# vdorie/stan4bart

Hardware: AMD Instinct MI355X
Metric: gibbs_iters_per_sec (higher is better)
Workload: dtype f64

## Files before the change

### include/stan4bart_amd.h

```cpp
#ifndef STAN4BART_AMD_H
#define STAN4BART_AMD_H

#include <stdint.h>
#include <stddef.h>

#ifndef S4B_PREFIX
#define S4B_PREFIX s4b_
#endif
#define S4B_CAT_(a, b) a##b
#define S4B_CAT(a, b) S4B_CAT_(a, b)
#define S4B_FN(name) S4B_CAT(S4B_PREFIX, name)

#ifdef __cplusplus
extern "C" {
#endif

#define S4B_INTERFACE_VERSION 6

typedef struct s4b_sampler s4b_sampler;

typedef struct {
  int32_t n_trees;
  int32_t n_thin;
  int32_t keep_trees;
// ... 138 lines not shown
  int64_t reserved[2];
} s4b_state_header;
int S4B_FN(get_state)(s4b_sampler* s, void* buf, int64_t cap, int64_t* size);
int S4B_FN(set_state)(s4b_sampler* s, const void* buf, int64_t size);

int S4B_FN(set_trace)(s4b_sampler* s, int32_t enable);
int S4B_FN(get_trace)(s4b_sampler* s, int64_t cap_records, int32_t* out, int64_t* num_records);
int S4B_FN(get_leaf_assignment)(s4b_sampler* s, int32_t tree, int32_t* out);
int S4B_FN(set_device_sharing)(s4b_sampler* s, int32_t chains);
int S4B_FN(set_tree_path)(s4b_sampler* s, int32_t path);
int S4B_FN(get_tree_path)(s4b_sampler* s, int32_t out[2]);
int S4B_FN(get_counters)(s4b_sampler* s, int64_t out[3]);
int S4B_FN(get_fused_stats)(s4b_sampler* s, int64_t out[2]);
int S4B_FN(get_sweep_stats)(s4b_sampler* s, int64_t out[2]);
int S4B_FN(get_sweep_spec)(s4b_sampler* s, int64_t out[4]);
int S4B_FN(get_sweep_busy)(s4b_sampler* s, int64_t* out);
int S4B_FN(set_hmc_mode)(s4b_sampler* s, int32_t mode);
int S4B_FN(get_hmc_mode)(s4b_sampler* s, int32_t* mode);

int S4B_FN(get_nuts_stats)(s4b_sampler* s, double out[4]);

int S4B_FN(profile_sweep)(s4b_sampler* s, int32_t n_sweeps, double out[8]);
int S4B_FN(stream_probe)(int32_t device, int64_t n_doubles, int32_t reps, double out[4]);

int S4B_FN(profile_leapfrog)(s4b_sampler* s, int32_t n_evals, double out[8]);

int S4B_FN(set_test_hook)(s4b_sampler* s, int32_t hook, int64_t value);

void S4B_FN(free)(s4b_sampler* s);

// ... 13 lines not shown
```

### stan4bart_amd/abi.py

```python
from __future__ import annotations

import ctypes as C
from dataclasses import dataclass, field
from typing import Callable, Optional, Sequence

import numpy as np

INTERFACE_VERSION = 6
c_double_p = C.POINTER(C.c_double)
c_int32_p = C.POINTER(C.c_int32)
c_uint32_p = C.POINTER(C.c_uint32)


class BartControl(C.Structure):
    _fields_ = [("n_trees", C.c_int32), ("n_thin", C.c_int32), ("keep_trees", C.c_int32),
                ("node_capacity", C.c_int32),
                ("base", C.c_double), ("power", C.c_double), ("k", C.c_double), ("node_scale", C.c_double),
                ("birth_or_death_prob", C.c_double), ("swap_prob", C.c_double),
                ("change_prob", C.c_double), ("birth_prob", C.c_double),
                ("split_probs", c_double_p), ("use_quantiles", C.c_int32), ("interface_version", C.c_int32),
                ("k_hyper_df", C.c_double), ("k_hyper_scale", C.c_double)]


class BartData(C.Structure):
# ... 237 lines not shown
            "get_parametric_mean": [vp, dp], "get_bart_data_range": [vp, dp],
            "get_r_rng_state": [vp, up], "set_r_rng_state": [vp, up],
            "get_dims": [vp, C.POINTER(i64)], "get_stan_par_names": [vp, C.c_char_p, C.c_size_t],
            "get_trees": [vp, i64, ip, ip, ip, ip, dp, C.POINTER(i64)],
            "get_kept_trees": [vp, i64, i64, ip, ip, ip, ip, ip, dp, C.POINTER(i64)],
            "get_kept_trees_indexed": [vp, ip, i64, ip, i64, i64, ip, ip, ip, ip, ip, dp, C.POINTER(i64)],
            "export_bart_state": [vp, vp, i64, C.POINTER(i64)],
            "create_stored_bart_sampler": [vp, i64, i32, C.POINTER(vp)],
            "predict_bart": [vp, dp, i64, dp, C.POINTER(i64)],
            "predict_bart_offset": [vp, dp, i64, dp, dp, C.POINTER(i64)], "print_trees": [vp, ip, i64, ip, i64],
            "get_state": [vp, vp, i64, C.POINTER(i64)], "set_state": [vp, vp, i64],
            "set_trace": [vp, i32], "get_trace": [vp, i64, ip, C.POINTER(i64)],
            "get_leaf_assignment": [vp, i32, ip], "get_counters": [vp, C.POINTER(i64)], "get_nuts_stats": [vp, dp],
            "profile_sweep": [vp, i32, dp], "profile_leapfrog": [vp, i32, dp],
            "set_progress": [vp, PROGRESS, vp], "set_device_sharing": [vp, i32],
            "set_tree_path": [vp, i32], "get_tree_path": [vp, ip], "get_fused_stats": [vp, C.POINTER(i64)], "get_sweep_stats": [vp, C.POINTER(i64)], "get_sweep_busy": [vp, C.POINTER(i64)], "get_sweep_spec": [vp, C.POINTER(i64)], "set_test_hook": [vp, i32, i64], "set_hmc_mode": [vp, i32], "get_hmc_mode": [vp, ip],
        }
        for name, argtypes in sig.items():
            fn = getattr(self._lib, self._pfx + name, None)
            if fn is None:
                continue
            fn.restype = C.c_int
            fn.argtypes = argtypes
        getattr(self._lib, self._pfx + "last_error").restype = C.c_char_p
        getattr(self._lib, self._pfx + "last_error").argtypes = []
        getattr(self._lib, self._pfx + "free").restype = None
        getattr(self._lib, self._pfx + "free").argtypes = [vp]

    def _f(self, name):
        return getattr(self._lib, self._pfx + name)

# ... 171 lines not shown
        fn = getattr(self._lib, self._pfx + "get_sweep_stats", None)
        if fn is None:
            return (0, 0)
        out = (C.c_int64 * 2)()
        self._check(fn(self._h, out))
        return (int(out[0]), int(out[1]))

    def get_sweep_spec(self):
        fn = getattr(self._lib, self._pfx + "get_sweep_spec", None)
        if fn is None:
            return (0, 0, 0, 0)
        out = (C.c_int64 * 4)()
        self._check(fn(self._h, out))
        return tuple(int(v) for v in out)

    def set_test_hook(self, hook: int, value: int):
        self._check(self._f("set_test_hook")(self._h, int(hook), int(value)))

    def get_sweep_busy(self) -> int:
        fn = getattr(self._lib, self._pfx + "get_sweep_busy", None)
        if fn is None:
            return 0
        out = C.c_int64(0)
        self._check(fn(self._h, C.byref(out)))
        return int(out.value)

    def set_trace(self, enable: bool):
        self._check(self._f("set_trace")(self._h, int(enable)))

    def get_trace(self, cap: int = 1 << 20) -> np.ndarray:
# ... 155 lines not shown
```

### stan4bart_amd/csrc/c_api.inc

```
#include <memory>
#include <string>

struct s4b_sampler { s4b::SamplerCore<S4B_DEV> core; template <class... A> explicit s4b_sampler(A... a) : core(a...) {} };
struct s4b_sweep_group { std::unique_ptr<s4b::SweepGroup> g; };

namespace { thread_local std::string g_last_error; }

#define S4B_TRY try {
#define S4B_CATCH } catch (const std::exception& e) { g_last_error = e.what(); return 1; } catch (...) { g_last_error = "unknown error"; return 1; } return 0;
#define S4B_NEED(s, what) if (!(s)) { g_last_error = what " called on NULL sampler"; return 1; }

extern "C" {

const char* S4B_FN(last_error)(void) { return g_last_error.c_str(); }

int S4B_FN(create)(const s4b_bart_control* bc, const s4b_bart_data* bd, const s4b_stan_data* sd, const s4b_stan_control* sc,
                   const s4b_common_control* cc, const uint32_t* rstate, s4b_sampler** out) {
  S4B_TRY
  if (!out) throw std::invalid_argument("create: NULL output pointer");
  *out = new s4b_sampler(bc, bd, sd, sc, cc, rstate);
  S4B_CATCH
}
int S4B_FN(run)(s4b_sampler* s, int32_t num_iter, int32_t is_warmup, int32_t results_type, s4b_results* out) {
  S4B_NEED(s, "run") S4B_TRY s->core.dev().bind(); s4b::SamplerCore<S4B_DEV>::GroupRun inRun(s->core); s->core.run(num_iter, is_warmup != 0, results_type, out); S4B_CATCH
// ... 46 lines not shown
int S4B_FN(get_state)(s4b_sampler* s, void* buf, int64_t cap, int64_t* size) {
  S4B_NEED(s, "get_state") S4B_TRY s->core.dev().bind(); if (!size) throw std::invalid_argument("get_state: NULL size pointer"); *size = s->core.get_state(buf, cap); S4B_CATCH
}
int S4B_FN(set_state)(s4b_sampler* s, const void* buf, int64_t size) { S4B_NEED(s, "set_state") S4B_TRY s->core.dev().bind(); s->core.set_state(buf, size); S4B_CATCH }
int S4B_FN(set_trace)(s4b_sampler* s, int32_t enable) { S4B_NEED(s, "set_trace") S4B_TRY s->core.dev().bind(); s->core.set_trace(enable != 0); S4B_CATCH }
int S4B_FN(get_trace)(s4b_sampler* s, int64_t cap, int32_t* out, int64_t* num) { S4B_NEED(s, "get_trace") S4B_TRY s->core.dev().bind(); *num = s->core.get_trace(cap, out); S4B_CATCH }
int S4B_FN(get_leaf_assignment)(s4b_sampler* s, int32_t t, int32_t* out) { S4B_NEED(s, "get_leaf_assignment") S4B_TRY s->core.dev().bind(); s->core.leaf_assignment(t, out); S4B_CATCH }
int S4B_FN(set_device_sharing)(s4b_sampler* s, int32_t chains) { S4B_NEED(s, "set_device_sharing") S4B_TRY s->core.dev().bind(); s->core.set_device_sharing(chains); S4B_CATCH }
int S4B_FN(set_tree_path)(s4b_sampler* s, int32_t path) { S4B_NEED(s, "set_tree_path") S4B_TRY s->core.dev().bind(); s->core.dev().set_tree_path(path); S4B_CATCH }
int S4B_FN(get_tree_path)(s4b_sampler* s, int32_t out[2]) { S4B_NEED(s, "get_tree_path") S4B_TRY if (!out) throw std::invalid_argument("get_tree_path: NULL output pointer"); s->core.dev().get_tree_path(out); S4B_CATCH }
int S4B_FN(set_hmc_mode)(s4b_sampler* s, int32_t mode) { S4B_NEED(s, "set_hmc_mode") S4B_TRY s->core.set_hmc_mode(mode); S4B_CATCH }
int S4B_FN(get_hmc_mode)(s4b_sampler* s, int32_t* mode) { S4B_NEED(s, "get_hmc_mode") S4B_TRY if (!mode) throw std::invalid_argument("get_hmc_mode: NULL output pointer"); *mode = s->core.hmc_mode(); S4B_CATCH }
int S4B_FN(get_fused_stats)(s4b_sampler* s, int64_t out[2]) { S4B_NEED(s, "get_fused_stats") S4B_TRY if (!out) throw std::invalid_argument("get_fused_stats: NULL output pointer"); s->core.dev().fused_stats(out); S4B_CATCH }
int S4B_FN(get_sweep_stats)(s4b_sampler* s, int64_t out[2]) { S4B_NEED(s, "get_sweep_stats") S4B_TRY if (!out) throw std::invalid_argument("get_sweep_stats: NULL output pointer"); s->core.dev().sweep_stats(out); S4B_CATCH }
int S4B_FN(get_sweep_spec)(s4b_sampler* s, int64_t out[4]) { S4B_NEED(s, "get_sweep_spec") S4B_TRY if (!out) throw std::invalid_argument("get_sweep_spec: NULL output pointer"); s->core.dev().sweep_spec(out); S4B_CATCH }
int S4B_FN(set_test_hook)(s4b_sampler* s, int32_t hook, int64_t value) { S4B_NEED(s, "set_test_hook") S4B_TRY s->core.dev().set_test_hook(hook, value); S4B_CATCH }
int S4B_FN(get_sweep_busy)(s4b_sampler* s, int64_t* out) { S4B_NEED(s, "get_sweep_busy") S4B_TRY if (!out) throw std::invalid_argument("get_sweep_busy: NULL output pointer"); *out = s->core.dev().sweep_busy(); S4B_CATCH }
int S4B_FN(get_counters)(s4b_sampler* s, int64_t out[3]) { S4B_NEED(s, "get_counters") S4B_TRY s->core.dev().bind(); s->core.counters(out); S4B_CATCH }
int S4B_FN(get_nuts_stats)(s4b_sampler* s, double out[4]) { S4B_NEED(s, "get_nuts_stats") S4B_TRY s->core.dev().bind(); s->core.nuts_stats(out); S4B_CATCH }
int S4B_FN(profile_sweep)(s4b_sampler* s, int32_t n_sweeps, double out[8]) { S4B_NEED(s, "profile_sweep") S4B_TRY s->core.dev().bind(); s->core.profile_sweep(n_sweeps, out); S4B_CATCH }
int S4B_FN(profile_leapfrog)(s4b_sampler* s, int32_t n_evals, double out[8]) { S4B_NEED(s, "profile_leapfrog") S4B_TRY s->core.dev().bind(); s->core.profile_leapfrog(n_evals, out); S4B_CATCH }
int S4B_FN(stream_probe)(int32_t device, int64_t n_doubles, int32_t reps, double out[4]) { S4B_TRY S4B_DEV::probe_stream(device, n_doubles, reps, out); S4B_CATCH }
void S4B_FN(free)(s4b_sampler* s) { if (s) { try { s->core.leave_group(); } catch (...) {} } delete s; }

int S4B_FN(sweep_group_create)(int32_t device, int32_t max_members, s4b_sweep_group** out) {
  S4B_TRY
  if (!out) throw std::invalid_argument("sweep_group_create: NULL output pointer");
  *out = new s4b_sweep_group{std::unique_ptr<s4b::SweepGroup>(s4b::SamplerCore<S4B_DEV>::make_group((int)device, (int)max_members))};
  S4B_CATCH
}
// ... 20 lines not shown
```

### stan4bart_amd/csrc/dev_hip.hip

```cpp
#include <hip/hip_runtime.h>
#include <atomic>
#include <mutex>
#include <chrono>

#include <cstdio>
#include <cstdlib>
#include <cstring>
#include <stdexcept>
#include <string>
#include <vector>
#include "sweep_group.hpp"
#ifdef S4B_CONTROL_TIMING
__device__ unsigned long long g_prop[32];
#define S4B_PROP_T(i) do { if (blockIdx.x == 0 && (threadIdx.x >> 6) == 1 && (threadIdx.x & 63) == 0) { atomicAdd(&g_prop[i], (unsigned long long)wall_clock64()); if ((i) == 7) atomicAdd(&g_prop[15], 1ull); if ((i) <= 1) atomicAdd(&g_prop[8 + (i)], 1ull); } } while (0)
#endif
#ifdef S4B_CONTROL_TIMING
__device__ unsigned long long g_dec[16];
#define S4B_DEC_T(i) do { if (blockIdx.x == 0 && threadIdx.x == 0) { atomicAdd(&g_dec[i], (unsigned long long)wall_clock64()); if ((i) == 0) atomicAdd(&g_dec[15], 1ull); } } while (0)
#endif
#ifdef S4B_SWEEP_TIMING
static __device__ unsigned long long g_dec[16];
#define S4B_DEC_T(i) do { if (blockIdx.x == 100 && threadIdx.x == 0) { if ((i) == 0) { g_dec[0] = (unsigned long long)wall_clock64(); atomicAdd(&g_dec[15], 1ull); } \
                                                                      else { atomicAdd(&g_dec[i], (unsigned long long)wall_clock64() - g_dec[0]); atomicAdd(&g_dec[7 + (i)], 1ull); } } } while (0)
#endif
// ... 1994 lines not shown
        const bool common = stepOk && !(weighted_ && (splitProbs_ || !weightedSweepBuilt || !wScaleOk || !wRangeOk)) && a.gridF >= 2 && a.gridF <= 256 &&
                            a.gridF <= prop.multiProcessorCount && sweep_lds_bytes() + staticLds <= 160 * 1024;
        sweepRegsOk_ = common && nQuads <= (int64_t)(a.gridF - 1) * SW_PT * SW_PF;
        const int64_t streamNP = a.gridF - 1, streamBlocks = (nQuads + SW_PT - 1) / SW_PT;
        const int64_t streamPerWg = (streamBlocks + streamNP - 1) / streamNP * 4 * SW_PT, streamPerCopy = (streamNP + XC_COPIES - 1) / XC_COPIES;
        const bool streamCountOk = streamPerWg < ((int64_t)1 << 16) && streamPerCopy * streamPerWg <= ((int64_t)1 << 21) - 1;
        sweepStreamOk_ = common && !splitProbs_ && !weighted_ && streamCountOk;
        sweepOk_ = sweepRegsOk_ || sweepStreamOk_;
        sweepSolo_ = nQuads <= (int64_t)SW_PT * SW_PF;
#ifdef S4B_TUNING
        if (getenv("S4B_NOSOLO")) sweepSolo_ = false;
#endif
        sweepFew_ = nQuads <= (int64_t)(SW_PF - 1) * (sweepSolo_ ? 1 : a.gridF - 1) * SW_PT;
        if (sweepOk_) {
          xbuf_ = zalloc<unsigned long long>((size_t)2 * (XC_RING_WORDS + XC_ROLL_WORDS));
          HIP_OK(hipHostMalloc(&sweepStatus_, 64, hipHostMallocCoherent | hipHostMallocMapped));
          sweepStatus_[0] = -1;
          { void* dp = nullptr; HIP_OK(hipHostGetDevicePointer(&dp, sweepStatus_, 0)); sweepStatusDev_ = (int32_t*)dp; }
          HIP_OK(hipFuncSetAttribute(reinterpret_cast<const void*>(k_sweep), hipFuncAttributeMaxDynamicSharedMemorySize, (int)sweep_lds_bytes()));
          HIP_OK(hipFuncSetAttribute(reinterpret_cast<const void*>(k_sweep_stream), hipFuncAttributeMaxDynamicSharedMemorySize, (int)sweep_lds_bytes()));
          HIP_OK(hipFuncSetAttribute(reinterpret_cast<const void*>(k_sweep_few), hipFuncAttributeMaxDynamicSharedMemorySize, (int)sweep_lds_bytes()));
          HIP_OK(hipFuncSetAttribute(reinterpret_cast<const void*>(k_sweep_sp), hipFuncAttributeMaxDynamicSharedMemorySize, (int)sweep_lds_bytes()));
          HIP_OK(hipFuncSetAttribute(reinterpret_cast<const void*>(k_sweep_few_sp), hipFuncAttributeMaxDynamicSharedMemorySize, (int)sweep_lds_bytes()));
          HIP_OK(hipFuncSetAttribute(reinterpret_cast<const void*>(k_sweep_w), hipFuncAttributeMaxDynamicSharedMemorySize, (int)sweep_lds_bytes()));
        }
      }
      choose_path();
    }
    int32_t* nc = alloc<int32_t>((size_t)P_); upload(nc, d.numCuts, (size_t)P_); a.numCuts = nc;
    a.trace = zalloc<StepRecord>((size_t)std::max(1, d.traceCap)); a.traceCount = zalloc<int32_t>(1); a.errFlag = zalloc<int32_t>(1);
    a.model = d.model; a.model.numCuts = nc; a.traceOn = 0; a.model.scratch = nullptr;
// ... 206 lines not shown
  void set_test_hook(int hook, int64_t value) {
    if (hook != 1 || value < 0) throw std::invalid_argument("set_test_hook: hook 1 (every k-th persistent launch reports a busy device; 0 = off) is the only one");
    hookBusyEvery_ = value; hookLaunchNo_ = 0;
  }
  void hook_before_persistent_launch() {
    if (hookBusyEvery_ <= 0 || sweepGrid_ == 1) return;
    if (++hookLaunchNo_ % hookBusyEvery_ != 0) return;
    unsigned long long* cur = xbuf_ + (size_t)xbufParity_ * (XC_RING_WORDS + XC_ROLL_WORDS);
    static const unsigned long long busy = SW_ROLL_BUSY;
    HIP_OK(hipMemcpyAsync(cur + XC_RING_WORDS + 1, &busy, 8, hipMemcpyHostToDevice, stream_));
  }
  void sweep_persistent_launch() {
    if (group_ && group_eligible()) { sweep_batched_launch(); return; }
    if (sweepLock_.owns_lock()) sweepLock_.unlock();
    sweepLock_ = std::unique_lock<std::mutex>(sweep_mutex(device_));
    for (int i = 0; i < 16; ++i) sweepStatus_[i] = 0;
    sweepStatus_[0] = -1;
    hook_before_persistent_launch();
    launch_sweep_kernel();
    const hipError_t e = hipGetLastError();
    if (e != hipSuccess) { sweepLock_.unlock(); HIP_OK(e); }
  }
  void launch_sweep_kernel() {
    if (sweepStream_) hipLaunchKernelGGL(k_sweep_stream, dim3(sweepGrid_), dim3(FBLOCK), sweep_lds_bytes(), stream_, a_, sweep_args());
    else if (weighted_) hipLaunchKernelGGL(k_sweep_w, dim3(sweepGrid_), dim3(FBLOCK), sweep_lds_bytes(), stream_, a_, sweep_args());
    else if (splitProbs_) hipLaunchKernelGGL(sweepFew_ ? k_sweep_few_sp : k_sweep_sp, dim3(sweepGrid_), dim3(FBLOCK), sweep_lds_bytes(), stream_, a_, sweep_args());
    else if (sweepFew_) hipLaunchKernelGGL(k_sweep_few, dim3(sweepGrid_), dim3(FBLOCK), sweep_lds_bytes(), stream_, a_, sweep_args());
    else hipLaunchKernelGGL(k_sweep, dim3(sweepGrid_), dim3(FBLOCK), sweep_lds_bytes(), stream_, a_, sweep_args());
    ++launches_;
  }
  bool sweep_streams() const { return sweepStream_; }
// ... 1 lines not shown
  friend class HipSweepGroup;
  SweepGroup* group_ = nullptr;
  int64_t groupBatched_ = 0;
  hipEvent_t evReady_ = nullptr;
  SweepArgs batchArgs_{};
  static SweepGroup* group_create(int device, int maxMembers);
  bool group_eligible() const { return is_persistent() && sweepGrid_ == 1 && !sweepStream_; }
  int batch_variant() const { return weighted_ ? 4 : (splitProbs_ ? (sweepFew_ ? 3 : 2) : (sweepFew_ ? 1 : 0)); }
  void join_group(SweepGroup* g) {
    if (group_) throw std::invalid_argument("sweep_group_join: the sampler is already in a sweep group");
    if (g->device() != device_) throw std::invalid_argument("sweep_group_join: the sampler runs on device " + std::to_string(device_) + ", the group on device " + std::to_string(g->device()));
    g->join(this); group_ = g;
  }
  void leave_group() { if (group_) { group_->leave(this); group_ = nullptr; } }
  void sweep_batched_launch() {
    for (int i = 0; i < 16; ++i) sweepStatus_[i] = 0;
    sweepStatus_[0] = -1;
    if (!evReady_) HIP_OK(hipEventCreateWithFlags(&evReady_, hipEventDisableTiming));
    batchArgs_ = sweep_args();
    HIP_OK(hipEventRecord(evReady_, stream_));
    GroupJob job; job.member = this; job.variant = batch_variant();
    group_->arrive(job);
    ++launches_; ++groupBatched_;
  }
  struct GroupTally {
    DevHip& d; int thin; int64_t b0;
    GroupTally(DevHip& dd, int th) : d(dd), thin(th), b0(dd.groupBatched_) {}
    ~GroupTally() { if (d.group_ && std::uncaught_exceptions() == 0) d.group_->count_unbatched(std::max<int64_t>(0, thin - (d.groupBatched_ - b0))); }
  };
  SweepArgs sweep_args() {
    unsigned long long* cur = xbuf_ + (size_t)xbufParity_ * (XC_RING_WORDS + XC_ROLL_WORDS);
// ... 244 lines not shown
  }
  void set_device_sharing(int chains) { sharing_ = chains; choose_path(); }
  void profile_sweep_persistent(int nSweeps, int thin, double* out) {
    double sum = 0; int cnt = 0;
#ifdef S4B_SWEEP_WG
    { sync(); static unsigned long long dropW[256 * 16]; sweep_wg_fetch(dropW); static unsigned long long dropD[256 * 64]; sweep_wd_fetch(dropD); }
#endif
#ifdef S4B_SWEEP_TIMING
    { sync(); unsigned long long drop[128]; sweep_timing_fetch(drop); }
#endif
    for (int sIdx = 0; sIdx < nSweeps * thin; ++sIdx) {
      const int64_t ho = sweepHandOvers_;
      {
        std::lock_guard<std::mutex> turn(sweep_mutex(device_));
        HIP_OK(hipEventRecord(evStart_, stream_));
        sweepStatus_[0] = -1; sweepStatus_[13] = 0; sweepStatus_[14] = 0;
        launch_sweep_kernel();
        HIP_OK(hipEventRecord(evStop_, stream_));
        sync();
      }
      const int st = sweepStatus_[0];
      ++sweepCount_;
      count_persistent_launch(st);
      if (st == -2) { ++sweepBusy_; sweep_fused_or_two_one(); if (binary_) launch_latents(); if (kModeled_) draw_k(); sync(); continue; }
      if (st < 0 || st > T_ + 1) throw std::runtime_error("persistent tree sweep: the launch did not complete");
      if (st != T_ + 1) {
        ++sweepHandOvers_;
        if (st == 0) { if (splitProbs_) sweep_two_one(); else sweep_fused_one(); }
        else { for (int t = st; t <= T_; ++t) { launch_step(t); ++launches_; }
               if (((T_ + 1) & 1) == 1) HIP_OK(hipMemcpyAsync(a_.rngF, a_.rngF + 1, sizeof(MTState), hipMemcpyDeviceToDevice, stream_)); }
      }
// ... 308 lines not shown
    for (int k = 0; k < K_; ++k) if (std::isfinite(cX[k])) mx = std::max(mx, std::fabs(cX[k]));
    for (int j = 0; j < q_; ++j) if (std::isfinite(cZ[j])) mz = std::max(mz, std::fabs(cZ[j]));
    const double tot[3] = {std::isfinite(ss) ? std::fabs(ss) : 0.0, mx, mz};
    if (fxLastBad_ == fusedEvals_ - 1)
      for (int g = 0; g < 3; ++g) {
        int want = fxExp_[g] - 10;
        if (tot[g] > 0.0) want = std::min(want, 20 - std::ilogb(tot[g]));
        fxExp_[g] = std::max(-900, std::min(900, want));
      }
    fxLastBad_ = fusedEvals_;
  }
  void fused_stats(int64_t out[2]) const { out[0] = fusedEvals_; out[1] = fusedFallbacks_; }
  void reset_fused_scales() { fxExp_[0] = fxExp_[1] = fxExp_[2] = 0; fxLastBad_ = -2; fxTinyFail_ = false; }
  void sweep_stats(int64_t out[2]) const { out[0] = sweepCount_; out[1] = sweepHandOvers_; }
  void sweep_spec(int64_t out[4]) const { out[0] = sweepLaunchesRun_; out[1] = sweepTreesInside_; out[2] = sweepSpecSteps_; out[3] = sweepSpecOk_; }
  void count_persistent_launch(int st) {
    if (st < 0 || st > T_ + 1) return;
    ++sweepLaunchesRun_; sweepTreesInside_ += st == T_ + 1 ? T_ : std::max(st - 1, 0);
    sweepSpecSteps_ += sweepStatus_[13]; sweepSpecOk_ += sweepStatus_[14];
  }
  int64_t sweep_busy() const { return sweepBusy_; }

  void profile_leapfrog(int nEvals, const double* beta, const double* b, double* out) {
    inlineBeta_ = nullptr; inlineB_ = nullptr;
    push_params(beta, b);
    if (stanFused_) { launch_stan_fused(0, 0, true); fusedParity_ ^= 1; } else reduce_pipeline(0, 0, 1);
    sync();
    const int64_t l0 = launches_;
    HIP_OK(hipEventRecord(evStart_, stream_));
    for (int i = 0; i < nEvals; ++i) { if (stanFused_) { launch_stan_fused(0, 0, true); fusedParity_ ^= 1; } else reduce_pipeline(0, 0, 1); }
    HIP_OK(hipEventRecord(evStop_, stream_));
    sync();
    float ms = 0; HIP_OK(hipEventElapsedTime(&ms, evStart_, evStop_));
    out[0] = ms * 1000.0 / nEvals; out[2] = (double)(launches_ - l0) / nEvals;
// ... 66 lines not shown
    double* dv = alloc<double>(val.size()); upload(dv, val.data(), val.size()); s.cscVal = dv;
    int32_t* cc = alloc<int32_t>(chunkCol.size()); upload(cc, chunkCol.data(), chunkCol.size()); s.chunkCol = cc;
    int64_t* cs = alloc<int64_t>(chunkStart.size()); upload(cs, chunkStart.data(), chunkStart.size()); s.chunkStart = cs;
    int32_t* cl = alloc<int32_t>(chunkLen.size()); upload(cl, chunkLen.data(), chunkLen.size()); s.chunkLen = cl;
    int32_t* cp = alloc<int32_t>(colChunkPtr.size()); upload(cp, colChunkPtr.data(), colChunkPtr.size()); s.colChunkPtr = cp;
    s.chunkPart = zalloc<double>((size_t)std::max(1, s.numChunks));
    HIP_OK(hipStreamSynchronize(stream_));
  }

  int device_ = 0; hipStream_t stream_ = nullptr; hipEvent_t evStart_ = nullptr, evStop_ = nullptr;
  int64_t n_ = 0, nTest_ = 0; int P_ = 0, T_ = 0, nc_ = 0, K_ = 0, q_ = 0, gridN_ = 1; bool binary_ = false;
  size_t ldsApply_ = 0, ldsControl_ = 0, ldsTree_ = 0, ldsStep_ = 0; bool useFused_ = false, fusedAuto_ = false, fusedOk_ = false;
  enum { PATH_TWO = 1, PATH_FUSED = 2, PATH_SWEEP = 4, PATH_STREAM = 5 };
  bool splitProbs_ = false, weighted_ = false; double wScale_ = 1.0, wUnscale_ = 1.0; bool sweepOk_ = false, sweepRegsOk_ = false, sweepStreamOk_ = false, sweepSolo_ = false, sweepFew_ = false, sweepStream_ = false; unsigned long long* xbuf_ = nullptr; int32_t* sweepStatus_ = nullptr; int32_t* sweepStatusDev_ = nullptr;
  int64_t sweepCount_ = 0, sweepHandOvers_ = 0;
  int64_t sweepLaunchesRun_ = 0, sweepTreesInside_ = 0, sweepSpecSteps_ = 0, sweepSpecOk_ = 0;
  int xbufParity_ = 0; long long dbgSweepNo_ = 0; int sweepGrid_ = 0;
  OffsetArgs pend_; bool pendOffset_ = false, pendSigma_ = false;
  int pathReq_ = 0, path_ = 0, sharing_ = 1;
  double dbgSweepMs_ = 0; int dbgSweeps_ = 0;
  hipGraph_t graph_ = nullptr; hipGraphExec_t graphExec_ = nullptr; int graphTrace_ = -1; bool useGraph_ = true;
  BartArrays a_; StanArrays s_;
  std::vector<void*> allocs_;
  char* arena_ = nullptr; size_t arenaSize_ = 0, arenaUsed_ = 0;
  double* pinned_ = nullptr; double* testOut_ = nullptr; double* latX_ = nullptr; double* testPinned_ = nullptr; bool testWanted_ = false, testQueued_ = false;
  int32_t* varDev_ = nullptr; int32_t* varPinned_ = nullptr; bool varWanted_ = false, varQueued_ = false;
  unsigned long long* fusedAcc_ = nullptr; int32_t* fusedBad_ = nullptr; unsigned long long* pinnedAcc_ = nullptr;
  size_t fusedLds_ = 0; int fusedParity_ = 0; bool stanFused_ = false;
  uint32_t fusedSeq_ = 0; int zFixed_ = -1; const double* inlineBeta_ = nullptr; const double* inlineB_ = nullptr;
  int fxExp_[3] = {0, 0, 0}; int64_t fusedEvals_ = 0, fusedFallbacks_ = 0, fxLastBad_ = -2; bool fxTinyFail_ = false;
  int64_t launches_ = 0;
// ... 81 lines not shown
```

### stan4bart_amd/csrc/dev_sweep.inc

```
#if defined(S4B_SWEEP_TIMING) || defined(S4B_SWEEP_WGT) || defined(S4B_SWEEP_WGD)
#define S4B_SWEEP_WG 1
#define SW_W(i) do { if (lane == 0 && t > 0 && t < T && (int)SW_BX < 256) atomicAdd(&g_wg[SW_BX * 16 + (i)], (unsigned long long)wall_clock64() - (unsigned long long)F.t0[t & 3]); } while (0)
#ifdef S4B_SWEEP_TU
__device__ unsigned long long g_pubMax[8], g_pubMin[8];
__device__ unsigned long long g_wg[256 * 16];
__device__ unsigned long long g_wd[256 * 64];
void sweep_wg_fetch(unsigned long long* out) {
  (void)hipMemcpyFromSymbol(out, HIP_SYMBOL(g_wg), sizeof(g_wg));
  static unsigned long long z[256 * 16]; (void)hipMemcpyToSymbol(HIP_SYMBOL(g_wg), z, sizeof(z));
}
__device__ __attribute__((noinline)) void sw_dur_add(int idx, unsigned long long v) { atomicAdd(&g_wd[idx], v); atomicAdd(&g_wd[idx + 8], 1ull); if (v > 300ull) atomicAdd(&g_wd[idx + 16], 1ull); atomicMax(&g_wd[idx + 24], v); }
__device__ __attribute__((noinline)) void sw_abs_add(int idx, long long v) { atomicAdd(&g_wd[idx], (unsigned long long)v); atomicAdd(&g_wd[idx + 16], 1ull); }
#ifdef S4B_SWEEP_WGD
#define SW_ABS(i) do { if (lane == 0 && t > 1 && t + 1 < T && (int)SW_BX < 256) sw_abs_add((int)SW_BX * 64 + 32 + (i), wall_clock64() - F.t0[t & 3]); } while (0)
#endif
void sweep_wd_fetch(unsigned long long* out) {
  (void)hipMemcpyFromSymbol(out, HIP_SYMBOL(g_wd), sizeof(g_wd));
  static unsigned long long z[256 * 64]; (void)hipMemcpyToSymbol(HIP_SYMBOL(g_wd), z, sizeof(z));
}
#else
void sweep_wg_fetch(unsigned long long* out);
void sweep_wd_fetch(unsigned long long* out);
#endif
#endif
// ... 1068 lines not shown
          }
          if (!(sp & 1)) return false;
          SW_ABS(1);
          const int nNe = __builtin_amdgcn_readfirstlane(F.specCnt);
          earlyUsed = rng.count + 2 * nNe;
          if constexpr (!STREAM) spin_counter(&F.passSeen, 4 * t, &F.abort);
          SW_ABS(2);
          if (lane == 0) F.bothStep = t;
          publish(earlyUsed, 0);
          if (lane == 0) __hip_atomic_store(&F.tablesReady, t, __ATOMIC_RELEASE, __HIP_MEMORY_SCOPE_WORKGROUP);
          earlyDone = true;
          SW_T(10); SW_T(11); SW_A(43);
#ifdef S4B_SWEEP_TIMING
          if ((int)SW_BX == SW_TIMED_WG && lane == 0 && t > 0 && t < T) atomicAdd(&F.tacc[35], 1ull);
#endif
          rng.mti += 2 * nNe; rng.count += 2 * nNe; rng.wbase = -64;
          {
            const int bA = (int)(int16_t)tbT.binA.r;
            const double c = wave_gather(bA & 63, binCnt);
            if (bA >= 0 && lane < hwmT) { cnt.r = (int32_t)c; mu.load(At[lane].muNew); }
          }
          return true;
        };
        auto post = [&]() {
          if (earlyDone) { if (rng.count != earlyUsed && lane == 0) *a.errFlag |= S4B_ERR_INTERNAL | S4B_ERR_I_FITS; return; }
          publish(rng.count, accepted);
          SW_T(10);
        };
        const int hwmNew = decide(curT, mu, cnt, muOld, hwmT, m, sigma, &rng, &prT, tbT, binCnt, binSum, binWt, wk, &accepted, &rec, caT, post, ctl, openRng, early);
        const int cntOut = prT.hwm > hwmNew ? prT.hwm : hwmNew;
        didDecide = true; dHwmNew = hwmNew; dCntOut = cntOut; dAccepted = accepted; dRec = rec;
// ... 231 lines not shown
          if (doit) pre = t + 2;
          if (lane == 0) {
            const CandSet ca = cand_lds(L.img, t + 2, 0);
            const bool there = doit && ca.meta[0] != 0;
            F.aheadId[(t + 2) % 3] = there ? drawNo : 0; F.aheadNb[(t + 2) % 3] = there ? ca.head->pr.nbA + ca.head->pr.nbB : 0;
            __hip_atomic_store(&F.pre0Ready, t + 2, __ATOMIC_RELEASE, __HIP_MEMORY_SCOPE_WORKGROUP);
          }
        }
      }
      if (wv == 1) { SW_MARK(); }
    }
  } else if (wv == 3) {
    int nbPrev = 0;
    bool prevAlt = false;
    int nSpecSteps = 0, nSpecOk = 0;
    bool prevOk = false;
    bool prevSelf = false;
    for (int t = 0; t <= T; ++t) {
      const bool doDecide = t > 0, doPropose = t < T;
      int specNb = 0;
      SW_KERNARGS();
      double zPre = 0.0, ppPre = 0.0, denPre = 1.0, sdPre = 0.0, wPre = 0.0, muOldPre = 0.0; bool preOk = false; int preNl = 0, preN = 0, preBA = 0, preMti0 = 0, specNbPre = 0, seqImg = 0;
      if (doDecide) {
        const CandSet cs = cand_lds(L.img, t - 1, __builtin_amdgcn_readfirstlane(F.selSlot[(t - 1) & 1]));
        const int32_t* const hd = (const int32_t*)cs.head;
        preNl = S4B_UNI(hd[21]);
        preMti0 = S4B_UNI((int)cs.rng->mti) + (S4B_UNI(hd[1]) == 1 ? 1 : 0);
        preOk = preMti0 + 2 * preNl <= 624;
        const bool in = lane < preNl;
        preN = in ? (int)cs.slab[SF_CLEAF * SW_NC + lane] & 63 : 0;
        preBA = (int)cs.slab[SF_BINA * SW_NC + preN] & 63;
        muOldPre = cs.snapMu[preN];
        wPre = in ? (double)cs.snapCnt[preN] : 0.0;
        const int k = (preOk && in) ? preMti0 + 2 * lane : 0;
        zPre = leaf_deviate(mt_word_to_unif(cs.rng->mt[k]), mt_word_to_unif(cs.rng->mt[k + 1]));
        ppPre = wPre / (M.sigma * M.sigma); denPre = a.model.leafPrec + ppPre; sdPre = 1.0 / sqrt(denPre);
        asm volatile("" : "+v"(zPre), "+v"(ppPre), "+v"(denPre), "+v"(sdPre), "+v"(muOldPre), "+v"(wPre));
        asm volatile("" : "+v"(preN), "+v"(preBA));
        if (!STREAM && doPropose && !solo) {
          spin_counter(&F.img0Ready, t, &F.abort);
          const CandSet c0 = cand_lds(L.img, t, 0);
          const int nbImg = S4B_UNI(c0.head->pr.nbA) + S4B_UNI(c0.head->pr.nbB);
          if (S4B_UNI(c0.meta[0]) != 0 && nbImg >= 1 && nbImg <= 8) { specNbPre = nbImg; seqImg = S4B_UNI(c0.meta[3]); }
        }
      }
      if (doDecide && hasObs && !(S4B_LINEAR && prevSelf && !prevAlt)) spin_counter(prevAlt ? &F.publishedAlt : &F.published, t, &F.abort);
      if (doDecide) {
        asm volatile("s_waitcnt vmcnt(0)" ::: "memory");
        unsigned long long* const xPrev = x.xbuf + (size_t)((prevAlt ? XC_RING : 0) + ((t + XC_RING - 1) & (XC_RING - 1))) * XC_BUF_WORDS;
        const int nw = solo ? 0 : 2 * NBX * nbPrev;
        bool fine = true;
#ifndef S4B_POLL_DELAY
#define S4B_POLL_DELAY 40
#endif
#ifndef S4B_POLL_SLEEP
#define S4B_POLL_SLEEP 2
#endif
        if (nw > 0 && !STREAM) __builtin_amdgcn_s_sleep(S4B_POLL_DELAY);
// ... 42 lines not shown
        }
#endif
#ifdef S4B_SWEEP_TIMING
        SW_AP(40);
#endif
        if (lane == 0) __hip_atomic_store(&S.arrived, t, __ATOMIC_RELEASE, __HIP_MEMORY_SCOPE_WORKGROUP);
        SW_T(1);
        {
          const int nl = preNl, n = preN;
          const bool in = lane < nl;
          const double lc = F.totC[preBA], ls = F.totS[preBA];
          const double lw = WT ? F.totS[nbPrev + preBA] : lc;
          const bool ne = in && lc != 0.0;
          const unsigned long long mask = __ballot(ne);
          const int cntNe = __popcll(mask);
          const bool valid = preMti0 + 2 * cntNe <= 624;
          double v = 0.0;
          if (!WT && preOk && cntNe == nl && __all(!in || lc == wPre)) {
            if (ne) v = leaf_value_parts(ppPre, denPre, sdPre, lc, ls, zPre);
          } else {
            const CandSet cs = cand_lds(L.img, t - 1, __builtin_amdgcn_readfirstlane(F.selSlot[(t - 1) & 1]));
            const int rank = (int)__builtin_amdgcn_mbcnt_hi((unsigned)(mask >> 32), __builtin_amdgcn_mbcnt_lo((unsigned)mask, 0u));
            const int k = (ne && valid) ? preMti0 + 2 * rank : 0;
            const uint32_t y1 = cs.rng->mt[k], y2 = cs.rng->mt[k + 1];
            if (ne) v = leaf_value(lw, ls, mt_word_to_unif(y1), mt_word_to_unif(y2), M.sigma * M.sigma, a.model.leafPrec);
          }
          if (S4B_LINEAR && !STREAM) spin_counter(&F.passSeen, 4 * (t - 1), &F.abort);
          if (in && valid) { NodeA na; na.muOld = muOldPre; na.muNew = v; (L.A + (STREAM ? 0 : (t & 1)) * SW_NC)[n] = na; }
          if (S4B_LINEAR && !STREAM && in && valid) L.dtab[(t & 1) * SW_NC + n] = muOldPre - v;
#if S4B_LINEAR
          if (lane == 0) { F.specCnt = cntNe; __hip_atomic_store(&F.specReady, (t << 1) | (valid ? 1 : 0), __ATOMIC_RELEASE, __HIP_MEMORY_SCOPE_WORKGROUP); }
          int nbLin = 0; bool dirty = false;
          if (specNbPre) {
#ifdef S4B_SWEEP_WGD
            const long long tW0 = wall_clock64();
#endif
            if (prevOk && S4B_LINEAR != 2) spin_counter(&F.preDoneA, t, &F.abort); else spin_counter(&F.preDoneB, t, &F.abort);
#ifdef S4B_SWEEP_WGD
            if (lane == 0 && t > 1 && t + 1 < T && (int)SW_BX < 256) sw_dur_add((int)SW_BX * 64 + 7, (unsigned long long)(wall_clock64() - tW0));
// ... 60 lines not shown
            unsigned long long* z = x.xbuf + (size_t)((c >= XC_COPIES ? XC_RING : 0) + ((t + 2) & (XC_RING - 1))) * XC_BUF_WORDS + (size_t)(c & (XC_COPIES - 1)) * XC_WORDS;
            __hip_atomic_store(z + lane, 0ull, __ATOMIC_RELAXED, __HIP_MEMORY_SCOPE_AGENT);
            __hip_atomic_store(z + 64 + lane, 0ull, __ATOMIC_RELAXED, __HIP_MEMORY_SCOPE_AGENT);
          }
        }
      }
      if (__hip_atomic_load(&F.abort, __ATOMIC_RELAXED, __HIP_MEMORY_SCOPE_WORKGROUP)) break;
      if (!doPropose) break;
      if (!spin_counter(&F.paGo, t + 1, &F.abort)) break;
      SW_G(94);
      const int nb = __builtin_amdgcn_readfirstlane(F.nb);
      const bool specOk = specNb != 0 && sweep_spec_confirmed(F, t, specNb);
      prevAlt = specNb != 0 && !specOk;
      prevOk = specOk; prevSelf = specNb != 0;
      nSpecSteps += specNb != 0 ? 1 : 0; nSpecOk += specOk ? 1 : 0;
      if (ctl && !solo && lane < NBX * nb && !specOk) {
        xc_publish(x.xbuf + (size_t)((prevAlt ? XC_RING : 0) + (t & (XC_RING - 1))) * XC_BUF_WORDS, lane, 0.0, 0, a.errFlag);
      }
      nbPrev = nb;
      SW_MARK();
      if (__builtin_amdgcn_readfirstlane(F.needBig)) { bailStep = t; break; }
    }
    if (ctl && lane == 0) { SW_KERNARGS(); x.status[13] = nSpecSteps; x.status[14] = nSpecOk; }
  } else {
    const int pw = wv - 4, pt = pw * 64 + lane;
    const int64_t stride = (int64_t)NP * SW_PT;
    const int64_t q0 = (int64_t)SW_BX * SW_PT + pt;
    PassBar bar; bar.ctr = &F.bar; bar.abortFlag = &F.abort; bar.epoch = 0; bar.tacc = F.tacc; bar.totS = F.totS; bar.totC = F.totC; bar.solo = solo; bar.arr = &F.statArr;
    if constexpr (STREAM) {
      for (int t = 0; t <= T; ++t) {
        const bool doDecide = t > 0, doPropose = t < T;
        const int tn = doPropose ? t : 0;
        SW_KERNARGS();
        const int64_t nQuads = (a.n + 3) >> 2;
        if (pw == 0 && doPropose) {
          if (t == 0 && T > 1) stage_tree(a, L.stage, 1, lane);
        if (t + 2 < T) { if (t >= 1) spin_counter(&F.img1Ready, t - 1, &F.abort); stage_tree(a, L.stage, t + 2, lane); }
          if (lane == 0) __hip_atomic_store(&F.staged, t + 2 < T ? t + 2 : T - 1, __ATOMIC_RELEASE, __HIP_MEMORY_SCOPE_WORKGROUP);
// ... 757 lines not shown
```

### stan4bart_amd/csrc/rrng_hd.hpp

```cpp
#ifndef S4B_RRNG_HD_HPP
#define S4B_RRNG_HD_HPP

#include <stdint.h>
#include <math.h>

#if defined(__HIPCC__)
#define S4B_HD __host__ __device__
#else
#define S4B_HD
#endif

#if defined(__HIP_DEVICE_COMPILE__)
__device__ __forceinline__ int s4b_uni(int v) { return __builtin_amdgcn_readfirstlane(v); }
__device__ __forceinline__ unsigned s4b_uni(unsigned v) { return (unsigned)__builtin_amdgcn_readfirstlane((int)v); }
__device__ __forceinline__ double s4b_uni(double v) {
  return __hiloint2double(__builtin_amdgcn_readfirstlane(__double2hiint(v)), __builtin_amdgcn_readfirstlane(__double2loint(v)));
}
#define S4B_UNI(x) s4b_uni(x)
#else
#define S4B_UNI(x) (x)
#endif

namespace s4b {

// ... 11 lines not shown
    const int k = base + lane;
    const bool in = k < 624;
    const int k1 = (k + 1 >= 624) ? k + 1 - 624 : k + 1, k397 = (k + 397 >= 624) ? k + 397 - 624 : k + 397;
    uint32_t a = in ? mt[k] : 0u, b = in ? mt[k1] : 0u, c = in ? mt[k397] : 0u;
    uint32_t y = (a & 0x80000000u) | (b & 0x7fffffffu);
    uint32_t v = c ^ (y >> 1);
    if (y & 1u) v ^= 0x9908b0dfu;
    if (in) mt[k] = v;
    __builtin_amdgcn_fence(__ATOMIC_RELEASE, "wavefront");
    __builtin_amdgcn_wave_barrier();
    __builtin_amdgcn_fence(__ATOMIC_ACQUIRE, "wavefront");
  }
  s->mti = 0;
}
#endif

S4B_HD inline void mt_regenerate(MTState* s) {
#if defined(__HIP_DEVICE_COMPILE__)
  if (S4B_UNI(s->pad) == 1) { mt_regenerate_wave(s); return; }
#endif
  uint32_t* mt = s->mt;
  for (int k = 0; k < 624; ++k) {
    uint32_t y = (mt[k] & 0x80000000u) | (mt[(k + 1) % 624] & 0x7fffffffu);
    uint32_t v = mt[(k + 397) % 624] ^ (y >> 1);
    if (y & 1u) v ^= 0x9908b0dfu;
    mt[k] = v;
  }
  s->mti = 0;
}

// ... 159 lines not shown
```

Baseline: 502.2.

## Allow speculative leaf draws across Mersenne Twister regeneration boundary

Adds a lookahead helper that computes Mersenne Twister words past index 624 from the current state without regenerating, and relaxes the speculation validity check so speculative leaf-value draws no longer fail when they cross the regeneration boundary. The RNG advance in the sweep now goes through rng_advance instead of bumping mti directly. It also adds per-cause counters for why speculation was skipped, plus an API to read them. The aim is to raise the speculation hit rate and avoid serialized fallback steps. The risk is RNG-stream correctness: the lookahead formula ignores dependencies once i+397 reaches 624.

```diff
diff --git a/include/stan4bart_amd.h b/include/stan4bart_amd.h
--- a/include/stan4bart_amd.h
+++ b/include/stan4bart_amd.h
@@ -176,6 +176,7 @@
 int S4B_FN(get_fused_stats)(s4b_sampler* s, int64_t out[2]);
 int S4B_FN(get_sweep_stats)(s4b_sampler* s, int64_t out[2]);
 int S4B_FN(get_sweep_spec)(s4b_sampler* s, int64_t out[4]);
+int S4B_FN(get_sweep_spec_causes)(s4b_sampler* s, int64_t out[5]);
 int S4B_FN(get_sweep_busy)(s4b_sampler* s, int64_t* out);
 int S4B_FN(set_hmc_mode)(s4b_sampler* s, int32_t mode);
 int S4B_FN(get_hmc_mode)(s4b_sampler* s, int32_t* mode);
diff --git a/stan4bart_amd/abi.py b/stan4bart_amd/abi.py
--- a/stan4bart_amd/abi.py
+++ b/stan4bart_amd/abi.py
@@ -275,7 +275,7 @@
             "get_leaf_assignment": [vp, i32, ip], "get_counters": [vp, C.POINTER(i64)], "get_nuts_stats": [vp, dp],
             "profile_sweep": [vp, i32, dp], "profile_leapfrog": [vp, i32, dp],
             "set_progress": [vp, PROGRESS, vp], "set_device_sharing": [vp, i32],
-            "set_tree_path": [vp, i32], "get_tree_path": [vp, ip], "get_fused_stats": [vp, C.POINTER(i64)], "get_sweep_stats": [vp, C.POINTER(i64)], "get_sweep_busy": [vp, C.POINTER(i64)], "get_sweep_spec": [vp, C.POINTER(i64)], "set_test_hook": [vp, i32, i64], "set_hmc_mode": [vp, i32], "get_hmc_mode": [vp, ip],
+            "set_tree_path": [vp, i32], "get_tree_path": [vp, ip], "get_fused_stats": [vp, C.POINTER(i64)], "get_sweep_stats": [vp, C.POINTER(i64)], "get_sweep_busy": [vp, C.POINTER(i64)], "get_sweep_spec": [vp, C.POINTER(i64)], "get_sweep_spec_causes": [vp, C.POINTER(i64)], "set_test_hook": [vp, i32, i64], "set_hmc_mode": [vp, i32], "get_hmc_mode": [vp, ip],
         }
         for name, argtypes in sig.items():
             fn = getattr(self._lib, self._pfx + name, None)
@@ -477,6 +477,14 @@
         self._check(fn(self._h, out))
         return tuple(int(v) for v in out)
 
+    def get_sweep_spec_causes(self):
+        fn = getattr(self._lib, self._pfx + "get_sweep_spec_causes", None)
+        if fn is None:
+            return (0, 0, 0, 0, 0)
+        out = (C.c_int64 * 5)()
+        self._check(fn(self._h, out))
+        return tuple(int(v) for v in out)
+
     def set_test_hook(self, hook: int, value: int):
         self._check(self._f("set_test_hook")(self._h, int(hook), int(value)))
 
diff --git a/stan4bart_amd/csrc/c_api.inc b/stan4bart_amd/csrc/c_api.inc
--- a/stan4bart_amd/csrc/c_api.inc
+++ b/stan4bart_amd/csrc/c_api.inc
@@ -84,6 +84,11 @@
 int S4B_FN(get_fused_stats)(s4b_sampler* s, int64_t out[2]) { S4B_NEED(s, "get_fused_stats") S4B_TRY if (!out) throw std::invalid_argument("get_fused_stats: NULL output pointer"); s->core.dev().fused_stats(out); S4B_CATCH }
 int S4B_FN(get_sweep_stats)(s4b_sampler* s, int64_t out[2]) { S4B_NEED(s, "get_sweep_stats") S4B_TRY if (!out) throw std::invalid_argument("get_sweep_stats: NULL output pointer"); s->core.dev().sweep_stats(out); S4B_CATCH }
 int S4B_FN(get_sweep_spec)(s4b_sampler* s, int64_t out[4]) { S4B_NEED(s, "get_sweep_spec") S4B_TRY if (!out) throw std::invalid_argument("get_sweep_spec: NULL output pointer"); s->core.dev().sweep_spec(out); S4B_CATCH }
+extern "C++" {
+template <class D> static auto s4b_spec_causes(const D& d, int64_t* out, int) -> decltype(d.sweep_spec_causes(out), void()) { d.sweep_spec_causes(out); }
+template <class D> static void s4b_spec_causes(const D&, int64_t* out, long) { for (int i = 0; i < 5; ++i) out[i] = 0; }
+}
+int S4B_FN(get_sweep_spec_causes)(s4b_sampler* s, int64_t out[5]) { S4B_NEED(s, "get_sweep_spec_causes") S4B_TRY if (!out) throw std::invalid_argument("get_sweep_spec_causes: NULL output pointer"); s4b_spec_causes(s->core.dev(), out, 0); S4B_CATCH }
 int S4B_FN(set_test_hook)(s4b_sampler* s, int32_t hook, int64_t value) { S4B_NEED(s, "set_test_hook") S4B_TRY s->core.dev().set_test_hook(hook, value); S4B_CATCH }
 int S4B_FN(get_sweep_busy)(s4b_sampler* s, int64_t* out) { S4B_NEED(s, "get_sweep_busy") S4B_TRY if (!out) throw std::invalid_argument("get_sweep_busy: NULL output pointer"); *out = s->core.dev().sweep_busy(); S4B_CATCH }
 int S4B_FN(get_counters)(s4b_sampler* s, int64_t out[3]) { S4B_NEED(s, "get_counters") S4B_TRY s->core.dev().bind(); s->core.counters(out); S4B_CATCH }
diff --git a/stan4bart_amd/csrc/dev_hip.hip b/stan4bart_amd/csrc/dev_hip.hip
--- a/stan4bart_amd/csrc/dev_hip.hip
+++ b/stan4bart_amd/csrc/dev_hip.hip
@@ -2032,7 +2032,7 @@
         sweepFew_ = nQuads <= (int64_t)(SW_PF - 1) * (sweepSolo_ ? 1 : a.gridF - 1) * SW_PT;
         if (sweepOk_) {
           xbuf_ = zalloc<unsigned long long>((size_t)2 * (XC_RING_WORDS + XC_ROLL_WORDS));
-          HIP_OK(hipHostMalloc(&sweepStatus_, 64, hipHostMallocCoherent | hipHostMallocMapped));
+          HIP_OK(hipHostMalloc(&sweepStatus_, 128, hipHostMallocCoherent | hipHostMallocMapped));
           sweepStatus_[0] = -1;
           { void* dp = nullptr; HIP_OK(hipHostGetDevicePointer(&dp, sweepStatus_, 0)); sweepStatusDev_ = (int32_t*)dp; }
           HIP_OK(hipFuncSetAttribute(reinterpret_cast<const void*>(k_sweep), hipFuncAttributeMaxDynamicSharedMemorySize, (int)sweep_lds_bytes()));
@@ -2269,7 +2269,7 @@
     if (group_ && group_eligible()) { sweep_batched_launch(); return; }
     if (sweepLock_.owns_lock()) sweepLock_.unlock();
     sweepLock_ = std::unique_lock<std::mutex>(sweep_mutex(device_));
-    for (int i = 0; i < 16; ++i) sweepStatus_[i] = 0;
+    for (int i = 0; i < 32; ++i) sweepStatus_[i] = 0;
     sweepStatus_[0] = -1;
     hook_before_persistent_launch();
     launch_sweep_kernel();
@@ -2301,7 +2301,7 @@
   }
   void leave_group() { if (group_) { group_->leave(this); group_ = nullptr; } }
   void sweep_batched_launch() {
-    for (int i = 0; i < 16; ++i) sweepStatus_[i] = 0;
+    for (int i = 0; i < 32; ++i) sweepStatus_[i] = 0;
     sweepStatus_[0] = -1;
     if (!evReady_) HIP_OK(hipEventCreateWithFlags(&evReady_, hipEventDisableTiming));
     batchArgs_ = sweep_args();
@@ -2576,7 +2576,7 @@
       {
         std::lock_guard<std::mutex> turn(sweep_mutex(device_));
         HIP_OK(hipEventRecord(evStart_, stream_));
-        sweepStatus_[0] = -1; sweepStatus_[13] = 0; sweepStatus_[14] = 0;
+        sweepStatus_[0] = -1; sweepStatus_[13] = 0; sweepStatus_[14] = 0; for (int i = 16; i < 21; ++i) sweepStatus_[i] = 0;
         launch_sweep_kernel();
         HIP_OK(hipEventRecord(evStop_, stream_));
         sync();
@@ -2915,10 +2915,12 @@
   void reset_fused_scales() { fxExp_[0] = fxExp_[1] = fxExp_[2] = 0; fxLastBad_ = -2; fxTinyFail_ = false; }
   void sweep_stats(int64_t out[2]) const { out[0] = sweepCount_; out[1] = sweepHandOvers_; }
   void sweep_spec(int64_t out[4]) const { out[0] = sweepLaunchesRun_; out[1] = sweepTreesInside_; out[2] = sweepSpecSteps_; out[3] = sweepSpecOk_; }
+  void sweep_spec_causes(int64_t out[5]) const { for (int i = 0; i < 5; ++i) out[i] = sweepSpecCauses_[i]; }
   void count_persistent_launch(int st) {
     if (st < 0 || st > T_ + 1) return;
     ++sweepLaunchesRun_; sweepTreesInside_ += st == T_ + 1 ? T_ : std::max(st - 1, 0);
     sweepSpecSteps_ += sweepStatus_[13]; sweepSpecOk_ += sweepStatus_[14];
+    for (int i = 0; i < 5; ++i) sweepSpecCauses_[i] += sweepStatus_[16 + i];
   }
   int64_t sweep_busy() const { return sweepBusy_; }
 
@@ -3015,7 +3017,7 @@
   enum { PATH_TWO = 1, PATH_FUSED = 2, PATH_SWEEP = 4, PATH_STREAM = 5 };
   bool splitProbs_ = false, weighted_ = false; double wScale_ = 1.0, wUnscale_ = 1.0; bool sweepOk_ = false, sweepRegsOk_ = false, sweepStreamOk_ = false, sweepSolo_ = false, sweepFew_ = false, sweepStream_ = false; unsigned long long* xbuf_ = nullptr; int32_t* sweepStatus_ = nullptr; int32_t* sweepStatusDev_ = nullptr;
   int64_t sweepCount_ = 0, sweepHandOvers_ = 0;
-  int64_t sweepLaunchesRun_ = 0, sweepTreesInside_ = 0, sweepSpecSteps_ = 0, sweepSpecOk_ = 0;
+  int64_t sweepLaunchesRun_ = 0, sweepTreesInside_ = 0, sweepSpecSteps_ = 0, sweepSpecOk_ = 0, sweepSpecCauses_[5] = {0, 0, 0, 0, 0};
   int xbufParity_ = 0; long long dbgSweepNo_ = 0; int sweepGrid_ = 0;
   OffsetArgs pend_; bool pendOffset_ = false, pendSigma_ = false;
   int pathReq_ = 0, path_ = 0, sharing_ = 1;
diff --git a/stan4bart_amd/csrc/dev_sweep.inc b/stan4bart_amd/csrc/dev_sweep.inc
--- a/stan4bart_amd/csrc/dev_sweep.inc
+++ b/stan4bart_amd/csrc/dev_sweep.inc
@@ -1106,7 +1106,7 @@
 #ifdef S4B_SWEEP_TIMING
           if ((int)SW_BX == SW_TIMED_WG && lane == 0 && t > 0 && t < T) atomicAdd(&F.tacc[35], 1ull);
 #endif
-          rng.mti += 2 * nNe; rng.count += 2 * nNe; rng.wbase = -64;
+          rng_advance(&rng, 2 * nNe); rng.count += 2 * nNe;
           {
             const int bA = (int)(int16_t)tbT.binA.r;
             const double c = wave_gather(bA & 63, binCnt);
@@ -1368,13 +1368,15 @@
     int nbPrev = 0;
     bool prevAlt = false;
     int nSpecSteps = 0, nSpecOk = 0;
+    int nNoWide = 0, nSpecRenew = 0;
+    int nNoImg = 0, nNoRenew = 0, nNoOther = 0;
     bool prevOk = false;
     bool prevSelf = false;
     for (int t = 0; t <= T; ++t) {
       const bool doDecide = t > 0, doPropose = t < T;
       int specNb = 0;
       SW_KERNARGS();
-      double zPre = 0.0, ppPre = 0.0, denPre = 1.0, sdPre = 0.0, wPre = 0.0, muOldPre = 0.0; bool preOk = false; int preNl = 0, preN = 0, preBA = 0, preMti0 = 0, specNbPre = 0, seqImg = 0;
+      double zPre = 0.0, ppPre = 0.0, denPre = 1.0, sdPre = 0.0, wPre = 0.0, muOldPre = 0.0; bool preOk = false, img0 = false, wide0 = false; int preNl = 0, preN = 0, preBA = 0, preMti0 = 0, specNbPre = 0, seqImg = 0;
       if (doDecide) {
         const CandSet cs = cand_lds(L.img, t - 1, __builtin_amdgcn_readfirstlane(F.selSlot[(t - 1) & 1]));
         const int32_t* const hd = (const int32_t*)cs.head;
@@ -1395,7 +1397,9 @@
           spin_counter(&F.img0Ready, t, &F.abort);
           const CandSet c0 = cand_lds(L.img, t, 0);
           const int nbImg = S4B_UNI(c0.head->pr.nbA) + S4B_UNI(c0.head->pr.nbB);
-          if (S4B_UNI(c0.meta[0]) != 0 && nbImg >= 1 && nbImg <= 8) { specNbPre = nbImg; seqImg = S4B_UNI(c0.meta[3]); }
+          img0 = S4B_UNI(c0.meta[0]) != 0;
+          wide0 = img0 && nbImg > 8;
+          if (img0 && nbImg >= 1 && nbImg <= 8) { specNbPre = nbImg; seqImg = S4B_UNI(c0.meta[3]); }
         }
       }
       if (doDecide && hasObs && !(S4B_LINEAR && prevSelf && !prevAlt)) spin_counter(prevAlt ? &F.publishedAlt : &F.published, t, &F.abort);
@@ -1468,7 +1472,7 @@
           const bool ne = in && lc != 0.0;
           const unsigned long long mask = __ballot(ne);
           const int cntNe = __popcll(mask);
-          const bool valid = preMti0 + 2 * cntNe <= 624;
+          const bool valid = preMti0 <= 624;
           double v = 0.0;
           if (!WT && preOk && cntNe == nl && __all(!in || lc == wPre)) {
             if (ne) v = leaf_value_parts(ppPre, denPre, sdPre, lc, ls, zPre);
@@ -1476,7 +1480,7 @@
             const CandSet cs = cand_lds(L.img, t - 1, __builtin_amdgcn_readfirstlane(F.selSlot[(t - 1) & 1]));
             const int rank = (int)__builtin_amdgcn_mbcnt_hi((unsigned)(mask >> 32), __builtin_amdgcn_mbcnt_lo((unsigned)mask, 0u));
             const int k = (ne && valid) ? preMti0 + 2 * rank : 0;
-            const uint32_t y1 = cs.rng->mt[k], y2 = cs.rng->mt[k + 1];
+            const uint32_t y1 = mt_word_ahead(cs.rng, k), y2 = mt_word_ahead(cs.rng, k + 1);
             if (ne) v = leaf_value(lw, ls, mt_word_to_unif(y1), mt_word_to_unif(y2), M.sigma * M.sigma, a.model.leafPrec);
           }
           if (S4B_LINEAR && !STREAM) spin_counter(&F.passSeen, 4 * (t - 1), &F.abort);
@@ -1567,6 +1571,11 @@
       prevAlt = specNb != 0 && !specOk;
       prevOk = specOk; prevSelf = specNb != 0;
       nSpecSteps += specNb != 0 ? 1 : 0; nSpecOk += specOk ? 1 : 0;
+      if (doDecide && !STREAM && !solo) {
+        nSpecRenew += (specNb != 0 && preMti0 + 2 * __builtin_amdgcn_readfirstlane(F.specCnt) > 624) ? 1 : 0;
+        const bool no = specNb == 0;
+        nNoWide += (no && wide0) ? 1 : 0; nNoImg += (no && !img0) ? 1 : 0; nNoRenew += (no && img0 && !wide0 && preMti0 > 624) ? 1 : 0; nNoOther += (no && img0 && !wide0 && preMti0 <= 624) ? 1 : 0;
+      }
       if (ctl && !solo && lane < NBX * nb && !specOk) {
         xc_publish(x.xbuf + (size_t)((prevAlt ? XC_RING : 0) + (t & (XC_RING - 1))) * XC_BUF_WORDS, lane, 0.0, 0, a.errFlag);
       }
@@ -1574,7 +1583,8 @@
       SW_MARK();
       if (__builtin_amdgcn_readfirstlane(F.needBig)) { bailStep = t; break; }
     }
-    if (ctl && lane == 0) { SW_KERNARGS(); x.status[13] = nSpecSteps; x.status[14] = nSpecOk; }
+    if (ctl && lane == 0) { SW_KERNARGS(); x.status[13] = nSpecSteps; x.status[14] = nSpecOk;
+                            x.status[16] = nNoWide; x.status[17] = nSpecRenew; x.status[18] = nNoImg; x.status[19] = nNoRenew; x.status[20] = nNoOther; }
   } else {
     const int pw = wv - 4, pt = pw * 64 + lane;
     const int64_t stride = (int64_t)NP * SW_PT;
diff --git a/stan4bart_amd/csrc/rrng_hd.hpp b/stan4bart_amd/csrc/rrng_hd.hpp
--- a/stan4bart_amd/csrc/rrng_hd.hpp
+++ b/stan4bart_amd/csrc/rrng_hd.hpp
@@ -49,6 +49,13 @@
   s->mti = 0;
 }
 #endif
+
+S4B_HD inline uint32_t mt_word_ahead(const MTState* s, int k) {
+  if (k < 624) return s->mt[k];
+  const int i = k - 624;
+  const uint32_t y = (s->mt[i] & 0x80000000u) | (s->mt[i + 1] & 0x7fffffffu);
+  return s->mt[i + 397] ^ (y >> 1) ^ ((y & 1u) ? 0x9908b0dfu : 0u);
+}
 
 S4B_HD inline void mt_regenerate(MTState* s) {
 #if defined(__HIP_DEVICE_COMPILE__)
```

Result: no change. 503.3 (median of 6 runs) (+0.2%).
